# Megvii-CSG/MegReader

Measured on AMD Instinct MI355X. Metric: training images/sec, CRNN-CTC 32x128 crops, batch 256 per GPU, higher is better.
Workload: dtype bf16; 1 GPU; CRNN + 1D-CTC training step (BASELINE.json configs[1]): 32x128 crops, T=33, C=38, Adam; global_batch=256, per_gpu_batch=256, parallelism=dp1, launch=hipGraph replay

## Files before the change

include/megreader_hip.h:

```cpp
#ifndef MEGREADER_HIP_H
#define MEGREADER_HIP_H

#include <hip/hip_runtime_api.h>

#ifdef __cplusplus
extern "C" {
#endif

#define MR_ABI_VERSION 3
#define MR_DTYPE_F32 0
#define MR_DTYPE_BF16 1

const char* mr_last_error(void);
int mr_abi_version(void);
int mr_phase_timer(int on);
int mr_phase_read(int id, double* total_ms, double* total_work);
int mr_init(void);

typedef struct mr_tuning {
  int nt_variant;
  int nt_deep;
  int nt_big;
  int nt_p8;
  int nt_force_bm;
// ... 48 lines not shown
                int NA, int NB, int row_perm_h, float* colsum, float* colsum2, hipStream_t stream);

int mr_tn_defer(int on);
int mr_tn_pending(void);
int mr_tn_discard(void);
int mr_tn_flush(hipStream_t stream);
int mr_tn_flush_beside(hipStream_t stream);

int mr_conv2d_fwd(int dtype, const void* x, const void* w_krsc, const float* bias, void* y, int relu, int Nimg,
                  int H, int W, int Cin, int ldx, int Cout, int ldy, int R, int S, int sh, int sw, int ph, int pw,
                  int dh, int dw, int Ho, int Wo, hipStream_t stream);
int mr_conv2d_fwd_pool_ok(int dtype, int Nimg, int H, int W, int Cin, int ldx, int Cout, int R, int S, int sh, int sw, int ph, int pw,
                          int dh, int dw, int Ho, int Wo, int pkh, int pkw, int psh, int psw, int pph, int ppw);
int mr_conv2d_fwd_pool(int dtype, const void* x, const void* w_krsc, const float* bias, void* y_pool, unsigned char* idx, int relu,
                       int Nimg, int H, int W, int Cin, int ldx, int Cout, int R, int S, int sh, int sw, int ph, int pw, int dh,
                       int dw, int Ho, int Wo, int pkh, int pkw, int psh, int psw, int pph, int ppw, int PHo, int PWo,
                       hipStream_t stream);
int mr_conv2d_fwd_stats(int dtype, const void* x, const void* w_krsc, const float* bias, void* y, double* bn_sums, int Nimg,
                        int H, int W, int Cin, int ldx, int Cout, int R, int S, int sh, int sw, int ph, int pw, int dh,
                        int dw, int Ho, int Wo, hipStream_t stream);
int mr_conv2d_dgrad(int dtype, const void* dy, const void* w_crsk, void* dx, int Nimg, int H, int W, int Cin,
                    int lddx, int Cout, int lddy, int R, int S, int sh, int sw, int ph, int pw, int dh, int dw,
                    int Ho, int Wo, hipStream_t stream);
int mr_conv2d_dgrad_add(int dtype, const void* dy, const void* w_crsk, void* dx, const void* addend, int Nimg, int H, int W,
                        int Cin, int lddx, int Cout, int lddy, int R, int S, int sh, int sw, int ph, int pw, int dh, int dw,
                        int Ho, int Wo, hipStream_t stream);
int mr_conv2d_dgrad_bnb(int dtype, const void* dy, const void* w_crsk, void* dx, const void* addend, const void* bn_x,
                        const void* bn_y, const float* bn_mean, const float* bn_rstd, double* bn_sums, int* produced,
                        int Nimg, int H, int W, int Cin, int lddx, int Cout, int lddy, int R, int S, int sh, int sw, int ph,
                        int pw, int dh, int dw, int Ho, int Wo, hipStream_t stream);
int mr_conv2d_wgrad(int dtype, const void* dy, const void* x, float* dw_krsc, float* dbias, int Nimg, int H, int W,
                    int Cin, int ldx, int Cout, int lddy, int R, int S, int sh, int sw, int ph, int pw, int dh,
                    int dw, int Ho, int Wo, hipStream_t stream);
int mr_conv2d_wgrad_tab(int dtype, const void* dy, const void* x, float* dw_krsc, float* dbias, int N, int H, int W,
                        int Cin, int ldx, int Cout, int lddy, int R, int S, int sh, int sw, int ph, int pw, int dh,
                        int dw, int Ho, int Wo, void* rowtab, int build, hipStream_t stream);

long long mr_db_loss_ws_bytes(void);
int mr_db_head_tail_fwd(int dtype, const void* xb, const void* xt, float* binary, float* thresh, float* tbinary, long long n,
                        float k, hipStream_t stream);
int mr_db_head_tail_bwd(int dtype, const float* binary, const float* thresh, const float* tbinary, const float* gb,
                        const float* gt, const float* gtb, void* dxb, void* dxt, long long n, float k, hipStream_t stream);
int mr_db_loss_fwd(const float* binary, const float* thresh, const float* tbinary, const float* gt, const float* mask,
                   const float* tmap, const float* tmask, float* negloss, void* ws, float* out, int N, long long HW,
                   float negative_ratio, float eps, float l1_scale, float bce_scale, hipStream_t stream);
int mr_db_loss_bwd(const float* binary, const float* thresh, const float* tbinary, const float* gt, const float* mask,
// ... 380 lines not shown
```

megreader_amd/backbones/crnn.py:

```python
import torch.nn as nn

from ..nn import Conv2d, BatchNorm2d, MaxPool2d, FusedReLU
from ..nn import functional as F


class _Stem(nn.Sequential):

    def forward(self, input):
        conv, pool = self[0][0], self[1]
        if F.stem_eligible(input, conv.weight, conv.stride, conv.padding, conv.dilation, _pair(pool.kernel_size),
                           _pair(pool.stride), _pair(pool.padding)):
            return F.stem_conv_relu_pool(input, conv.weight, conv.bias)
        return super().forward(input)


class _ConvReluPool(nn.Sequential):

    def forward(self, input):
        conv, pool = self[0][0], self[1]
        if F.conv_relu_pool_eligible(input, conv.weight, conv.stride, conv.padding, conv.dilation, _pair(pool.kernel_size),
                                     _pair(pool.stride), _pair(pool.padding)):
            return F.conv_relu_pool(input, conv.weight, conv.bias, conv.padding, _pair(pool.kernel_size), _pair(pool.stride),
                                    _pair(pool.padding))
        return super().forward(input)
# ... 5 lines not shown

class CRNN(nn.Module):

    def __init__(self, imgH, nc, nclass, nh):
        super(CRNN, self).__init__()
        assert imgH % 16 == 0, 'imgH has to be a multiple of 16'

        self.kernels = [3, 3, 3, 3, 3, 3, 2]
        self.paddings = [1, 1, 1, 1, 1, 1, 0]
        self.strides = [1, 1, 1, 1, 1, 1, 1]
        self.channels = [64, 128, 256, 256, 512, 512, 512, nc]

        conv0 = _Stem(self._make_layer(0, pooled=True), MaxPool2d((2, 2), relu_input=True))
        conv1 = _ConvReluPool(self._make_layer(1, pooled=True), MaxPool2d((2, 2), relu_input=True))
        conv2 = self._make_layer(2, True)
        conv3 = _ConvReluPool(self._make_layer(3, pooled=True), MaxPool2d((2, 2), (2, 1), (0, 1), relu_input=True))
        conv4 = self._make_layer(4, True)
        conv5 = _ConvReluPool(self._make_layer(5, pooled=True), MaxPool2d((2, 2), (2, 1), (0, 1), relu_input=True))
        conv6 = self._make_layer(6, True)

        self.cnn = nn.Sequential(conv0, conv1, conv2, conv3, conv4, conv5, conv6)
        conv3[0][0].sole_consumer_of_bn = True
        conv5[0][0].sole_consumer_of_bn = True

    def _make_layer(self, i, batch_normalization=False, pooled=False):
        in_channel = self.channels[i - 1]
        out_channel = self.channels[i]
        layer = list()
        layer.append(Conv2d(in_channel, out_channel, self.kernels[i], self.strides[i], self.paddings[i],
                            fuse_relu=not batch_normalization,
                            relu_grad_downstream=pooled and not batch_normalization))
        if batch_normalization:
            layer.append(BatchNorm2d(out_channel))
        else:
            layer.append(FusedReLU())
        return nn.Sequential(*layer)

    def forward(self, input):
        return self.cnn(input)


def crnn_backbone(imgH=32, nc=3, nclass=37, nh=256):
    return CRNN(imgH, nc, nclass, nh)
```

megreader_amd/csrc/gemm_conv.hip:

```cpp
#include "igemm_core.h"
#include "igemm_p8.h"
#include "tn_taps.h"
#include "nt32.h"
#include "device.h"
#include "../../include/megreader_hip.h"

#include <algorithm>
#include <mutex>
#include <vector>

namespace mr {

static bool aligned16(const void* p) { return (((uintptr_t)p) & 15) == 0; }

#define g_nt_variant MR_TUNE(nt_variant)
#define g_nt_deep MR_TUNE(nt_deep)

struct BnbRequest { const void* x; const void* y; const float* mean; const float* rstd; };
struct NtEpilogue {
  const float* bias = nullptr;
  int relu = 0;
  const void* addend = nullptr;
  double* stats = nullptr;
  BnbRequest bnb = {nullptr, nullptr, nullptr, nullptr};
// ... 560 lines not shown
  }
  const TileChoice tw = nt_tile(M, N);
  if (tw.bm == 128 && tw.bn == 128 && (MR_TUNE(nt_wide8) & 1) && N % 128 == 0) {
    const int t = fit(128);
    if (t == 128) { *tile_rows = t; return 8; }
  }
  return 0;
}

template <int WM, int WN, int TM, int TN>
static int launch_nt_pool(const NtArgs& a, const ConvGeom& g, const EpiPool<bf16_t>& epi, hipStream_t stream) {
  constexpr int BM = WM * TM * 16, BN = WN * TN * 16;
  constexpr size_t lds_stage = 2 * (size_t)(BM + BN) * 128, lds_tile = (size_t)BM * BN * 2;
  constexpr size_t lds = lds_stage > lds_tile ? lds_stage : lds_tile;
  auto kern = igemm_nt_big_kernel<bf16_t, WM, WN, TM, TN, 2, EpiPool<bf16_t>>;
  if (const int rc = ensure_dynamic_lds(kern, lds)) return rc;
  const int tiles_m = cdiv(a.M, a.tile_rows), tiles_n = cdiv(a.N, BN);
  const int grid = cdiv(tiles_m, 8) * 8 * tiles_n;
  hipLaunchKernelGGL(kern, dim3(grid), dim3(64 * WM * WN), lds, stream, a, g, epi);
  MR_CHECK_LAUNCH();
  return MR_OK;
}


extern "C" {

int mr_init(void) {
  const int rc = tuning_from_env();
  if (rc != MR_OK) return rc;
  if (!zero_page()) { set_error("mr_init: zero page allocation failed"); return MR_ERR_LAUNCH; }
  return MR_OK;
}

#ifdef MR_ABLATION
int mr_set_tn_abl(int mask) {
  const int old = g_tn_abl;
  g_tn_abl = mask;
  return old;
}
int mr_set_tn_taps_abl(int mask) { return taps_set_abl(mask); }
#endif

int mr_set_tn_taps_workspace(void* ws, long long bytes) {
  MR_CHECK_ARG((ws == nullptr) == (bytes == 0) && bytes >= 0 && (((uintptr_t)ws) & 15) == 0,
               "mr_set_tn_taps_workspace: bad workspace");
  taps_set_workspace(ws, bytes);
// ... 184 lines not shown
                        hipStream_t stream) {
  MR_CHECK_ARG(dtype == MR_F32 || dtype == MR_BF16, "mr_conv2d_dgrad: bad dtype %d", dtype);
  const int vec = dtype == MR_F32 ? 4 : 8;
  MR_CHECK_ARG(Cout % vec == 0 && lddy % vec == 0, "mr_conv2d_dgrad: Cout/lddy must be multiples of %d", vec);
  MR_CHECK_ARG(aligned16(dy) && aligned16(w_crsk), "mr_conv2d_dgrad: dy and w must be 16-byte aligned");
  NtArgs a;
  a.A = dy; a.B = w_crsk; a.M = Nimg * H * W; a.N = Cin; a.K = R * S * Cout; a.lda = 0; a.ldb = R * S * Cout; a.zero = nullptr;
  ConvGeom g;
  fill_geom(g, 2, Ho, Wo, Cout, lddy, H, W, R, S, sh, sw, ph, pw, dh, dw);
  if (R * S <= 32 && sh == 1 && sw == 1) {
    if (dtype == MR_F32) return dispatch_nt_store<float, 2>(a, g, dx, lddx, o, stream);
    return dispatch_nt_store<bf16_t, 2>(a, g, dx, lddx, o, stream);
  }
  if (dtype == MR_F32) return dispatch_nt_store<float, 1>(a, g, dx, lddx, o, stream);
  return dispatch_nt_store<bf16_t, 1>(a, g, dx, lddx, o, stream);
}
int mr_conv2d_dgrad(int dtype, const void* dy, const void* w_crsk, void* dx, int Nimg, int H, int W, int Cin,
                    int lddx, int Cout, int lddy, int R, int S, int sh, int sw, int ph, int pw, int dh, int dw,
                    int Ho, int Wo, hipStream_t stream) {
  NtEpilogue o;
  return conv2d_dgrad(dtype, dy, w_crsk, dx, o, Nimg, H, W, Cin, lddx, Cout, lddy, R, S, sh, sw, ph, pw, dh, dw, Ho, Wo, stream);
}

int mr_conv2d_dgrad_add(int dtype, const void* dy, const void* w_crsk, void* dx, const void* addend, int Nimg, int H, int W,
                        int Cin, int lddx, int Cout, int lddy, int R, int S, int sh, int sw, int ph, int pw, int dh, int dw,
                        int Ho, int Wo, hipStream_t stream) {
  NtEpilogue o;
  o.addend = addend;
  return conv2d_dgrad(dtype, dy, w_crsk, dx, o, Nimg, H, W, Cin, lddx, Cout, lddy, R, S, sh, sw, ph, pw, dh, dw, Ho, Wo, stream);
}

int mr_conv2d_dgrad_bnb(int dtype, const void* dy, const void* w_crsk, void* dx, const void* addend, const void* bn_x,
                        const void* bn_y, const float* bn_mean, const float* bn_rstd, double* bn_sums, int* produced,
                        int Nimg, int H, int W, int Cin, int lddx, int Cout, int lddy, int R, int S, int sh, int sw, int ph,
                        int pw, int dh, int dw, int Ho, int Wo, hipStream_t stream) {
  MR_CHECK_ARG(bn_x && bn_mean && bn_rstd && bn_sums && produced, "mr_conv2d_dgrad_bnb: null BatchNorm operand");
  MR_CHECK_ARG(lddx == Cin, "mr_conv2d_dgrad_bnb: dx must be dense (lddx == Cin), like the BatchNorm's tensors");
  MR_CHECK_ARG(aligned16(bn_x) && (bn_y == nullptr || aligned16(bn_y)), "mr_conv2d_dgrad_bnb: bn_x / bn_y must be 16-byte aligned");
  NtEpilogue o;
  o.addend = addend;
  o.stats = bn_sums;
  o.bnb = BnbRequest{bn_x, bn_y, bn_mean, bn_rstd};
  const int rc = conv2d_dgrad(dtype, dy, w_crsk, dx, o, Nimg, H, W, Cin, lddx, Cout, lddy, R, S, sh, sw, ph, pw, dh, dw, Ho, Wo,
                              stream);
  *produced = o.stats_missed ? 0 : 1;
  return rc;
// ... 57 lines not shown
```

megreader_amd/csrc/igemm_core.h:

```cpp
#pragma once
#include "common.h"
#include <type_traits>

namespace mr {

struct ConvGeom {
  int Hg, Wg, Cg, ldg;
  int Hm, Wm;
  int R, S, sh, sw, ph, pw, dh, dw;
  int mode;
};

__device__ __forceinline__ bool conv_src(const ConvGeom& g, int hm, int wm, int r, int s, int& hi, int& wi) {
  if (g.mode == 1) {
    hi = hm * g.sh - g.ph + r * g.dh;
    wi = wm * g.sw - g.pw + s * g.dw;
  } else {
    int hn = hm + g.ph - r * g.dh;
    int wn = wm + g.pw - s * g.dw;
    if (hn < 0 || wn < 0) return false;
    if (g.sh == 1 && g.sw == 1) {
      hi = hn;
      wi = wn;
    } else {
// ... 18 lines not shown
#pragma unroll
    for (int j = 0; j < 4; ++j) acc = __builtin_amdgcn_mfma_f32_16x16x4f32(a[j], b[j], acc, 0, 0, 0);
  }
};

struct NtArgs {
  const void* A;
  const void* B;
  int M, N, K;
  long long lda;
  int ldb;
  const void* zero;
  int m_begin = 0;
  int ksplit = 1;
  void* ws = nullptr;
  int tile_rows = 0;
};
constexpr int NT_SPLIT_TICKETS = 4096;

__device__ __forceinline__ uint4 ldg16(const void* p) { return *(const uint4*)p; }

template <typename Epi> struct EpiHasStats { static constexpr bool value = false; };
template <typename Epi> struct EpiIsPool { static constexpr bool value = false; };
__device__ __forceinline__ float row16_sum(float v) {
#define MR_ROW_ROR(V, N) __builtin_bit_cast(float, __builtin_amdgcn_update_dpp(0, __builtin_bit_cast(int, V), 0x120 + (N), 0xf, 0xf, false))
  v += MR_ROW_ROR(v, 8);
  v += MR_ROW_ROR(v, 4);
  v += MR_ROW_ROR(v, 2);
  v += MR_ROW_ROR(v, 1);
#undef MR_ROW_ROR
  return v;
}
template <typename T, int CNT> struct EpiColStats {
  float s[4 * CNT], q[4 * CNT];
  __device__ __forceinline__ void init() {
#pragma unroll
    for (int e = 0; e < 4 * CNT; ++e) s[e] = q[e] = 0.f;
  }
  template <typename Epi> __device__ __forceinline__ void add(const Epi& epi, int m, int n, const f32x4* v) {
    if (m >= epi.M) return;
    if constexpr (Epi::kBnb) {
      const long long row = (long long)m * epi.ldc + n;
#pragma unroll
      for (int i = 0; i < CNT; ++i)
#pragma unroll
        for (int j = 0; j < 4; ++j) {
// ... 1192 lines not shown
                  }
                  first = false;
                }
            }
          T o[8];
#pragma unroll
          for (int e = 0; e < 8; ++e) o[e] = from_f32<T>(best[e]);
          const long long q = (((long long)nimg * epi.PHo + h / kh) * epi.PWo + pwi) * epi.ldc + n0 + c * 8;
          *(uint4*)(epi.C + q) = *(const uint4*)o;
          *(uint2*)(epi.idx + q) = *(const uint2*)bi;
        }
        pwi += PSTEP;
        while (pwi >= epi.PWo) {
          pwi -= epi.PWo;
          ++pr;
          h += kh;
          if (h >= epi.Ho) { h -= epi.Ho; ++nimg; }
        }
      }
    };
    if (epi.kh == 2 && epi.kw == 2) pool_one(std::integral_constant<int, 2>{}, std::integral_constant<int, 2>{});
    else pool_one(std::integral_constant<int, 0>{}, std::integral_constant<int, 0>{});
    return;
  } else {
    constexpr bool FLAGSHIP = (WM == 2 && WN == 4 && TM == 8 && TN == 4) || (WM == 1 && WN == 8 && TM == 17 && TN == 2);
    constexpr int EPI_PATHS = FLAGSHIP ? NT_EPI_STORE : (TN == 2 && !(WM == 4 && TM == 3)) ? (NT_EPI_PLAIN | NT_EPI_ADD) : 0;
    if constexpr (EPI_PATHS != 0) {
      if (nt_epilogue_interior<T, TM, TN, EPI_PATHS>(epi, m0 + wm_ * WTM, n0 + wn_ * WTN, l15, lg,
                                                      [&](int i, int j) -> f32x4 { return acc[i][j]; }))
        return;
    }
  EpiColStats<T, TN> cst;
  bool with_stats = false;
  if constexpr (EpiHasStats<Epi>::value) with_stats = epi.stats != nullptr;
  if (with_stats) cst.init();
#pragma unroll
  for (int j = 0; j < TM; ++j) {
    f32x4 run[TN];
#pragma unroll
    for (int i = 0; i < TN; ++i) run[i] = acc[i][j];
    if constexpr (EpiHasStats<Epi>::value)
      if (with_stats) cst.add(epi, m0 + wm_ * WTM + j * 16 + l15, n0 + wn_ * WTN + lg * (4 * TN), run);
    epi.template store_run<TN>(m0 + wm_ * WTM + j * 16 + l15, n0 + wn_ * WTN + lg * (4 * TN), run);
  }
  if constexpr (EpiHasStats<Epi>::value)
    if (with_stats) cst.flush(epi, n0 + wn_ * WTN + lg * (4 * TN), l15);
  }
}

template <typename T> struct EpiPool {
  T* C;
  unsigned char* idx;
  long long ldc;
  const float* bias;
  int relu;
  int M, N;
  int Nimg, Ho, Wo, kh, kw, sw, pw, PHo, PWo;
};
template <typename T> struct EpiIsPool<EpiPool<T>> { static constexpr bool value = true; };

template <typename T> struct EpiStore {
  T* C;
  long long ldc;
  const float* bias;
  int relu;
  int M, N;
  int vec_ok;
  double* stats = nullptr;
  int stats_ncopy = 1;
  const T* addend = nullptr;
  static constexpr bool kBnb = false;
  __device__ __forceinline__ void operator()(int m, int n, f32x4 v) const {
    if (m >= M || n >= N) return;
    if (bias) {
#pragma unroll
      for (int j = 0; j < 4; ++j)
        if (n + j < N) v[j] += bias[n + j];
    }
    if (addend) {
      const T* a = addend + (long long)m * ldc + n;
#pragma unroll
      for (int j = 0; j < 4; ++j)
// ... 932 lines not shown
```

megreader_amd/nn/functional.py:

```python
import ctypes
import os

import torch
from torch.autograd import Function

from .. import get_compute_dtype
from . import prep
from .._lib import call, dtype_code, load, ptr, require_cuda, vec_of

_ESIZE = {torch.float32: 4, torch.bfloat16: 2}


def _ceil_to(x, m):
    return (x + m - 1) // m * m


def grad_sink(param, physical_shape=None):
    sink = getattr(param, "_mr_grad_sink", None)
    if sink is None or sink.dtype != torch.float32 or not sink.is_cuda:
        return None
    if param.grad is None or param.grad.data_ptr() != sink.data_ptr():
        return None
    if physical_shape == "strided":
        return sink
# ... 264 lines not shown
    K, C, R, S = weight.shape
    dev = weight.device

    def build(old):
        if old is None:
            alloc = torch.zeros if Kp != K else torch.empty
            w_krsc = alloc((Kp, R, S, Cp), dtype=dtype, device=dev)
            w_crsk = alloc((C, R, S, Kp), dtype=dtype, device=dev) if need_dx else None
            bias_p = torch.zeros((Kp,), dtype=torch.float32, device=dev) if (bias is not None and Kp != K) else None
        else:
            w_krsc, w_crsk, bias_p = old
        jobs = [prep.conv_job(ptr(weight), weight.stride(), ptr(w_krsc), ptr(w_crsk), K, C, R, S, Cp, Kp)]
        if bias_p is not None:
            jobs.append(prep.bias_job(ptr(bias), 0, ptr(bias_p), K, 0))
        return (w_krsc, w_crsk, bias_p), jobs

    w_krsc, w_crsk, bias_p = prep.prepared((weight, bias), ("conv", Cp, Kp, bool(need_dx)), build, dtype)
    return w_krsc, w_crsk, (bias_p if bias_p is not None else bias)


class Conv2dFn(Function):
    @staticmethod
    def forward(ctx, x, weight, bias, stride, padding, dilation, relu, relu_grad_downstream=False, bn_sums=None,
                fork=False, bnb_link=None):
        require_cuda(x, weight, bias)
        ctx.bnb_link = bnb_link
        dtype = get_compute_dtype()
        dt = dtype_code(dtype)
        v = vec_of(dtype)
        xi = to_internal(x, dtype)
        N, H, W, Cp = xi.shape
        K, C, R, S = weight.shape
        if C > Cp or weight.dtype != torch.float32:
            raise RuntimeError("conv weight %s does not match input channels %d" % (tuple(weight.shape), Cp))
        Kp = _ceil_to(K, v)
        sh, sw = stride
        ph, pw = padding
        dh, dw = dilation
        Ho, Wo = _conv_out(H, R, sh, ph, dh), _conv_out(W, S, sw, pw, dw)
        need_dx = ctx.needs_input_grad[0]
        if need_dx and Cp != C:
            raise RuntimeError("input gradient requested for a channel-padded convolution input")
        w_krsc, w_crsk, bias_k = _conv_operands(weight, bias, dtype, Cp, Kp, need_dx)
        y = torch.empty((N, Ho, Wo, Kp), dtype=dtype, device=x.device)
        if bn_sums is not None and not relu and Kp == K:
            call("mr_conv2d_fwd_stats", dt, ptr(xi), ptr(w_krsc), ptr(bias_k), ptr(y), ptr(bn_sums), N, H, W, Cp, Cp, Kp,
                 R, S, sh, sw, ph, pw, dh, dw, Ho, Wo)
        else:
            call("mr_conv2d_fwd", dt, ptr(xi), ptr(w_krsc), ptr(bias_k), ptr(y), int(relu), N, H, W, Cp, Cp, Kp, Kp, R,
# ... 27 lines not shown
            call("mr_relu_bwd", dt, ptr(g), ptr(y), ptr(gm), g.numel())
            g = gm
        dx = dwt = db = None
        if ctx.needs_input_grad[0]:
            dxi = torch.empty((N, H, W, C), dtype=dtype, device=g.device)
            ga = None
            if g_fork is not None:
                ga = _grad_internal(g_fork, dtype)
                if tuple(ga.shape) != (N, H, W, C) or not ga.is_contiguous():
                    ga = ga.contiguous()
            link = ctx.bnb_link
            fused_bnb = False
            if link is not None and link.xi is not None and link.dtype == dtype and tuple(link.xi.shape) == (N, H, W, C) and \
                    BNB_EPILOGUE:
                sums = ZeroArena.take(g.device, load().mr_bn_scratch_doubles(C))
                if sums is not None:
                    produced = ctypes.c_int(0)
                    call("mr_conv2d_dgrad_bnb", dt, ptr(g), ptr(w_crsk), ptr(dxi), ptr(ga), ptr(link.xi), ptr(link.y),
                         ptr(link.mean), ptr(link.rstd), ptr(sums), ctypes.byref(produced), N, H, W, C, C, Kp, Kp, R, S, sh,
                         sw, ph, pw, dh, dw, Ho, Wo)
                    fused_bnb = True
                    if produced.value:
                        link.sums, link.grad_ptr = sums, dxi.data_ptr()
            if fused_bnb:
                pass
            elif ga is not None:
                call("mr_conv2d_dgrad_add", dt, ptr(g), ptr(w_crsk), ptr(dxi), ptr(ga), N, H, W, C, C, Kp, Kp, R, S, sh, sw,
                     ph, pw, dh, dw, Ho, Wo)
            elif POINTWISE_STRIDED_DGRAD and R == 1 and S == 1 and (sh > 1 or sw > 1) and ph == 0 and pw == 0:
                dxs = torch.empty((N, Ho, Wo, C), dtype=dtype, device=g.device)
                call("mr_conv2d_dgrad", dt, ptr(g), ptr(w_crsk), ptr(dxs), N, Ho, Wo, C, C, Kp, Kp, 1, 1, 1, 1, 0, 0, 1, 1, Ho,
                     Wo)
                call("mr_scatter_strided", dt, ptr(dxs), ptr(dxi), N, H, W, C, sh, sw, Ho, Wo)
            else:
                call("mr_conv2d_dgrad", dt, ptr(g), ptr(w_crsk), ptr(dxi), N, H, W, C, C, Kp, Kp, R, S, sh, sw, ph, pw,
                     dh, dw, Ho, Wo)
            dx = dxi.permute(0, 3, 1, 2)
        elif g_fork is not None:
            raise RuntimeError("conv2d_fork: the forked input received a gradient but the convolution input needs none")
        weight_p, bias_p = ctx.params
        want_db = ctx.has_bias and ctx.needs_input_grad[2]
        w_sink = grad_sink(weight_p, (K, R, S, C)) if (ctx.needs_input_grad[1] and Cp == C) else None
        b_sink = grad_sink(bias_p, (K,)) if want_db else None
        Kw = K if (w_sink is not None or b_sink is not None) else Kp
        if want_db:
            db = b_sink if b_sink is not None else torch.zeros((Kp,), dtype=torch.float32, device=g.device)
        if ctx.needs_input_grad[1]:
            gw = w_sink if w_sink is not None else torch.zeros((Kp, R, S, Cp), dtype=torch.float32, device=g.device)
            tab, build = (None, 0)
            if dtype == torch.bfloat16 and R * S <= 32:
                tab, build = _wgrad_rowtab(g.device, (N, H, W, Cp, R, S, sh, sw, ph, pw, dh, dw, Ho, Wo), Kw % 8 == 0)
            def wgrad_launch():
                call("mr_conv2d_wgrad_tab", dt, ptr(g), ptr(xi), ptr(gw), ptr(db) if want_db else 0, N, H, W, Cp, Cp, Kw,
                     Kp, R, S, sh, sw, ph, pw, dh, dw, Ho, Wo, ptr(tab), build)
            if _wgrad(wgrad_launch, w_sink is not None and (not want_db or b_sink is not None), (g, xi, tab),
                      [weight_p] + ([bias_p] if want_db else [])):
                return dx, None, None, None, None, None, None, None, None, None, None
            if w_sink is not None:
                dwt = None
                notify_grad_ready(weight_p)
            else:
                if Cp != C or Kp != K:
                    gw = gw[:K, :, :, :C]
                dwt = gw.permute(0, 3, 1, 2)
        elif want_db:
            call("mr_colsum", dt, ptr(g), ptr(db), N * Ho * Wo, Kw, Kp, 0)
        if want_db:
            if b_sink is not None:
                db = None
                notify_grad_ready(bias_p)
            elif Kp != K:
                db = db[:K]
        return dx, dwt, db, None, None, None, None, None, None, None, None


POINTWISE_STRIDED_DGRAD = os.environ.get("MEGREADER_POINTWISE_STRIDED_DGRAD", "1") != "0"

BNB_EPILOGUE = os.environ.get("MEGREADER_BNB_EPILOGUE", "0") == "1"


_DIST_GUARD = {"done": False}


def _no_resident_grids_beside_collectives():
    if _DIST_GUARD["done"]:
        return
    import torch.distributed as dist
    if dist.is_available() and dist.is_initialized():
        from ..runtime import no_resident_grid_kernels_beside_collectives
        no_resident_grid_kernels_beside_collectives(dist.get_world_size())
        _DIST_GUARD["done"] = True


class BnBwdLink(object):
    __slots__ = ("xi", "y", "mean", "rstd", "dtype", "sums", "grad_ptr")

    def __init__(self):
        self.xi = self.y = self.mean = self.rstd = self.dtype = self.sums = self.grad_ptr = None


class BnStatsHandoff(object):
    __slots__ = ("sums", "data_ptr", "dtype", "P", "C")

    def __init__(self, sums, data_ptr, dtype, P, C):
        self.sums, self.data_ptr, self.dtype, self.P, self.C = sums, data_ptr, dtype, P, C


def conv2d(x, weight, bias=None, stride=(1, 1), padding=(0, 0), dilation=(1, 1), relu=False,
           relu_grad_downstream=False, bn_stats=False, fork=False, sole_consumer_of_bn=False):
    sums = None
    if bn_stats and not relu and x.is_cuda:
        K = weight.shape[0]
        if K % vec_of(get_compute_dtype()) == 0:
            sums = ZeroArena.take(x.device, load().mr_bn_scratch_doubles(K))
    want_fork = bool(fork)
    fork = want_fork and x.requires_grad and torch.is_grad_enabled()
    link = getattr(x, "_mr_bnb_link", None) if (sole_consumer_of_bn and x.requires_grad and torch.is_grad_enabled()) else None
    y = Conv2dFn.apply(x, weight, bias, tuple(stride), tuple(padding), tuple(dilation), bool(relu),
                       bool(relu_grad_downstream), sums, fork, link)
    x_fork = x
    if fork:
        y, x_fork = y
    if sums is not None:
        y._mr_bn_sums = BnStatsHandoff(sums, y.data_ptr(), get_compute_dtype(), y.shape[0] * y.shape[2] * y.shape[3],
                                       y.shape[1])
    return (y, x_fork) if want_fork else y


class BatchNormFn(Function):
    @staticmethod
    def forward(ctx, x, gamma, beta, running_mean, running_var, training, momentum, eps, relu, residual,
                num_batches_tracked=None, pre=None, link=None):
        require_cuda(x, gamma, beta)
        dtype = get_compute_dtype()
        dt = dtype_code(dtype)
        xi = to_internal(x, dtype)
        N, H, W, C = xi.shape
        if C != gamma.numel():
            raise RuntimeError("BatchNorm2d: channel mismatch (%d vs %d)" % (C, gamma.numel()))
        P = N * H * W
        ri = to_internal(residual, dtype) if residual is not None else None
        y = torch.empty_like(xi)
# ... 218 lines not shown
        if want_db:
            db = b_sink if b_sink is not None else torch.zeros((64,), dtype=torch.float32, device=g.device)
        if dw is not None or db is not None:
            ws = torch.empty((load().mr_stem_bwd_workspace(C),), dtype=torch.float32, device=g.device)
            sk, sc, sr, ss = dw.stride() if dw is not None else (0, 0, 0, 0)
            call("mr_stem_bwd", dtype_code(dtype), ptr(g), ptr(code), ptr(x), ptr(ws), ptr(dw), sk, sc, sr, ss, ptr(db),
                 N, C, H, W)
        if w_sink is not None:
            notify_grad_ready(weight_p)
            dw = None
        if b_sink is not None:
            notify_grad_ready(bias_p)
            db = None
        return None, dw, db


def stem_conv_relu_pool(x, weight, bias):
    return StemConvReluPoolFn.apply(x, weight, bias)


class ConvReluPoolFn(Function):

    @staticmethod
    def forward(ctx, x, weight, bias, padding, pool_kernel, pool_stride, pool_padding):
        require_cuda(x, weight, bias)
        dtype = get_compute_dtype()
        dt = dtype_code(dtype)
        xi = to_internal(x, dtype)
        N, H, W, Cp = xi.shape
        K, C, R, S = weight.shape
        ph, pw = padding
        Ho, Wo = _conv_out(H, R, 1, ph, 1), _conv_out(W, S, 1, pw, 1)
        kh, kw = pool_kernel
        psh, psw = pool_stride
        pph, ppw = pool_padding
        PHo, PWo = (Ho + 2 * pph - kh) // psh + 1, (Wo + 2 * ppw - kw) // psw + 1
        need_dx = ctx.needs_input_grad[0]
        w_krsc, w_crsk, bias_k = _conv_operands(weight, bias, dtype, Cp, K, need_dx)
        y = torch.empty((N, PHo, PWo, K), dtype=dtype, device=x.device)
        idx = torch.empty((N, PHo, PWo, K), dtype=torch.uint8, device=x.device)
        call("mr_conv2d_fwd_pool", dt, ptr(xi), ptr(w_krsc), ptr(bias_k), ptr(y), ptr(idx), 1, N, H, W, Cp, Cp, K, R, S, 1, 1, ph, pw,
             1, 1, Ho, Wo, kh, kw, psh, psw, pph, ppw, PHo, PWo)
        ctx.save_for_backward(xi, w_crsk, idx, y)
        ctx.params = (weight, bias)
        ctx.geom = (N, H, W, Cp, C, K, K, R, S, 1, 1, ph, pw, 1, 1, Ho, Wo)
        ctx.pool = (kh, kw, psh, psw, pph, ppw, PHo, PWo)
        ctx.has_bias = bias is not None
        ctx.dtype = dtype
        return y.permute(0, 3, 1, 2)

    @staticmethod
    def backward(ctx, gy):
        xi, w_crsk, idx, y = ctx.saved_tensors
        N, H, W, Cp, C, K, Kp, R, S, sh, sw, ph, pw, dh, dw, Ho, Wo = ctx.geom
        kh, kw, psh, psw, pph, ppw, PHo, PWo = ctx.pool
        dtype = ctx.dtype
        g = _grad_internal(gy, dtype)
        dz = torch.empty((N, Ho, Wo, K), dtype=dtype, device=g.device)
        call("mr_maxpool_bwd", dtype_code(dtype), ptr(g), ptr(idx), ptr(y), ptr(dz), N, Ho, Wo, K, kh, kw, psh, psw, pph, ppw,
             PHo, PWo)

        class _ConvCtx(object):
            pass
        c = _ConvCtx()
        c.saved_tensors = (xi, w_crsk, None)
        c.geom, c.dtype, c.params, c.has_bias = ctx.geom, dtype, ctx.params, ctx.has_bias
        c.relu, c.bnb_link = False, None
        c.needs_input_grad = (ctx.needs_input_grad[0], ctx.needs_input_grad[1], ctx.needs_input_grad[2]) + (False,) * 8
        grads = Conv2dFn.backward(c, dz.permute(0, 3, 1, 2))
        return grads[0], grads[1], grads[2], None, None, None, None


def conv_relu_pool_eligible(x, weight, stride, padding, dilation, pool_kernel, pool_stride, pool_padding):
    if not x.is_cuda or get_compute_dtype() != torch.bfloat16 or tuple(stride) != (1, 1) or tuple(dilation) != (1, 1):
        return False
    if os.environ.get("MEGREADER_CONV_POOL", "1") == "0":
        return False
    N, C, H, W = x.shape
    K, Cw, R, S = weight.shape
    if C != Cw or C % 8 != 0 or K % 8 != 0:
        return False
    ph, pw = padding
    Ho, Wo = _conv_out(H, R, 1, ph, 1), _conv_out(W, S, 1, pw, 1)
    return bool(load().mr_conv2d_fwd_pool_ok(dtype_code(torch.bfloat16), N, H, W, C, C, K, R, S, 1, 1, ph, pw, 1, 1, Ho, Wo,
                                             pool_kernel[0], pool_kernel[1], pool_stride[0], pool_stride[1],
                                             pool_padding[0], pool_padding[1]))


def conv_relu_pool(x, weight, bias, padding, pool_kernel, pool_stride, pool_padding):
    return ConvReluPoolFn.apply(x, weight, bias, tuple(padding), tuple(pool_kernel), tuple(pool_stride), tuple(pool_padding))


class MaxPoolFn(Function):
    @staticmethod
    def forward(ctx, x, kernel, stride, padding, relu_input=False):
        require_cuda(x)
        dtype = get_compute_dtype()
        dt = dtype_code(dtype)
        xi = to_internal(x, dtype)
        N, H, W, C = xi.shape
        kh, kw = kernel
        sh, sw = stride
        ph, pw = padding
        Ho, Wo = (H + 2 * ph - kh) // sh + 1, (W + 2 * pw - kw) // sw + 1
        y = torch.empty((N, Ho, Wo, C), dtype=dtype, device=x.device)
        idx = torch.empty((N, Ho, Wo, C), dtype=torch.uint8, device=x.device)
        call("mr_maxpool_fwd", dt, ptr(xi), ptr(y), ptr(idx), N, H, W, C, kh, kw, sh, sw, ph, pw, Ho, Wo)
        ctx.save_for_backward(idx, y if relu_input else None)
        ctx.geom = (N, H, W, C, kh, kw, sh, sw, ph, pw, Ho, Wo)
        ctx.dtype = dtype
        return y.permute(0, 3, 1, 2)

    @staticmethod
    def backward(ctx, gy):
        idx, relu_y = ctx.saved_tensors
        N, H, W, C, kh, kw, sh, sw, ph, pw, Ho, Wo = ctx.geom
        dtype = ctx.dtype
        g = _grad_internal(gy, dtype)
        dx = torch.empty((N, H, W, C), dtype=dtype, device=g.device)
        call("mr_maxpool_bwd", dtype_code(dtype), ptr(g), ptr(idx), ptr(relu_y), ptr(dx), N, H, W, C, kh, kw, sh, sw,
             ph, pw, Ho, Wo)
        return dx.permute(0, 3, 1, 2), None, None, None, None


def max_pool2d(x, kernel, stride=None, padding=(0, 0), relu_input=False):
    stride = kernel if stride is None else stride
    return MaxPoolFn.apply(x, tuple(kernel), tuple(stride), tuple(padding), bool(relu_input))


class MapToSequenceFn(Function):
    @staticmethod
    def forward(ctx, x):
        require_cuda(x)
        dtype = get_compute_dtype()
        xi = to_internal(x, dtype)
        N, H, W, C = xi.shape
        if H != 1:
            raise AssertionError("the height of conv must be 1")
        out = torch.empty((W, N, C), dtype=dtype, device=x.device)
        call("mr_permute_021", dtype_code(dtype), ptr(xi), ptr(out), N, W, C)
        ctx.shape = (N, W, C)
        ctx.dtype = dtype
        return out

    @staticmethod
    def backward(ctx, g):
        N, W, C = ctx.shape
        dtype = ctx.dtype
        if g.dtype != dtype or not g.is_contiguous():
            g = g.to(dtype).contiguous()
# ... 814 lines not shown
```

megreader_amd/nn/modules.py:

```python
import math

import torch
import torch.nn as nn

from . import functional as F


BN_EPILOGUE = __import__("os").environ.get("MEGREADER_BN_EPILOGUE", "1") != "0"


FORK_RESIDUAL = __import__("os").environ.get("MEGREADER_FORK_RESIDUAL", "1") != "0"


def _pair(v):
    return tuple(v) if isinstance(v, (tuple, list)) else (v, v)


class Conv2d(nn.Conv2d):

    def __init__(self, *args, fuse_relu=False, relu_grad_downstream=False, **kwargs):
        super().__init__(*args, **kwargs)
        if self.groups != 1 or self.padding_mode != "zeros" or isinstance(self.padding, str):
            raise NotImplementedError("megreader_amd.nn.Conv2d supports groups=1 and explicit zero padding only")
        self.fuse_relu = fuse_relu
        self.relu_grad_downstream = relu_grad_downstream and fuse_relu
        self.weight.data = self.weight.data.contiguous(memory_format=torch.channels_last)

    feeds_batch_norm = False
    sole_consumer_of_bn = False
    sole_consumer_when_forked = False

    def forward(self, x):
        y = F.conv2d(x, self.weight, self.bias, self.stride, self.padding, self.dilation, self.fuse_relu,
                     self.relu_grad_downstream, bn_stats=self.feeds_batch_norm and self.training and BN_EPILOGUE,
                     sole_consumer_of_bn=self.sole_consumer_of_bn)
        y._mr_producer = self
        return y

    def forward_fork(self, x):
        if not FORK_RESIDUAL:
            y = F.conv2d(x, self.weight, self.bias, self.stride, self.padding, self.dilation, self.fuse_relu,
                         self.relu_grad_downstream, bn_stats=self.feeds_batch_norm and self.training and BN_EPILOGUE)
            y._mr_producer = self
            return y, x
        y, xr = F.conv2d(x, self.weight, self.bias, self.stride, self.padding, self.dilation, self.fuse_relu,
                         self.relu_grad_downstream, bn_stats=self.feeds_batch_norm and self.training and BN_EPILOGUE,
                         fork=True, sole_consumer_of_bn=self.sole_consumer_when_forked)
        y._mr_producer = self
        return y, xr


class FusedReLU(nn.Module):

    def forward(self, x):
        return x


class BatchNorm2d(nn.BatchNorm2d):
# ... 80 lines not shown
```

Measured before the change: 109,800 images/s.

## Fuse maxpool backward scatter into the following conv's dgrad epilogue

Result: no change. 110,600 images/s (median of 6 runs) (+0.6%).

```diff
diff --git a/include/megreader_hip.h b/include/megreader_hip.h
--- a/include/megreader_hip.h
+++ b/include/megreader_hip.h
@@ -94,6 +94,14 @@
 int mr_conv2d_dgrad(int dtype, const void* dy, const void* w_crsk, void* dx, int Nimg, int H, int W, int Cin,
                     int lddx, int Cout, int lddy, int R, int S, int sh, int sw, int ph, int pw, int dh, int dw,
                     int Ho, int Wo, hipStream_t stream);
+int mr_set_dgrad_unpool(int on);
+int mr_conv2d_dgrad_unpool_ok(int dtype, int Nimg, int H, int W, int Cin, int lddx, int Cout, int lddy, int R, int S, int sh, int sw,
+                              int ph, int pw, int dh, int dw, int Ho, int Wo, int pkh, int pkw, int psh, int psw, int pph, int ppw,
+                              int H_full, int W_full);
+int mr_conv2d_dgrad_unpool(int dtype, const void* dy, const void* w_crsk, void* dx_full, const unsigned char* idx, const void* relu_y,
+                           int Nimg, int H, int W, int Cin, int lddx, int Cout, int lddy, int R, int S, int sh, int sw, int ph, int pw,
+                           int dh, int dw, int Ho, int Wo, int pkh, int pkw, int psh, int psw, int pph, int ppw, int H_full, int W_full,
+                           hipStream_t stream);
 int mr_conv2d_dgrad_add(int dtype, const void* dy, const void* w_crsk, void* dx, const void* addend, int Nimg, int H, int W,
                         int Cin, int lddx, int Cout, int lddy, int R, int S, int sh, int sw, int ph, int pw, int dh, int dw,
                         int Ho, int Wo, hipStream_t stream);
diff --git a/megreader_amd/backbones/crnn.py b/megreader_amd/backbones/crnn.py
--- a/megreader_amd/backbones/crnn.py
+++ b/megreader_amd/backbones/crnn.py
@@ -51,6 +51,9 @@
         self.cnn = nn.Sequential(conv0, conv1, conv2, conv3, conv4, conv5, conv6)
         conv3[0][0].sole_consumer_of_bn = True
         conv5[0][0].sole_consumer_of_bn = True
+        conv2[0].sole_consumer_of_pool = True
+        conv4[0].sole_consumer_of_pool = True
+        conv6[0].sole_consumer_of_pool = True
 
     def _make_layer(self, i, batch_normalization=False, pooled=False):
         in_channel = self.channels[i - 1]
diff --git a/megreader_amd/csrc/gemm_conv.hip b/megreader_amd/csrc/gemm_conv.hip
--- a/megreader_amd/csrc/gemm_conv.hip
+++ b/megreader_amd/csrc/gemm_conv.hip
@@ -606,6 +606,46 @@
   return MR_OK;
 }
 
+static int g_dgrad_unpool = 1;
+
+static int dgrad_unpool_plan(int M, int N, int K, int Cg, int PWo, int* tile_rows) {
+  if (!__atomic_load_n(&g_dgrad_unpool, __ATOMIC_RELAXED) || g_nt_variant != 2 || forced_tile().bm || (Cg % 64) != 0 ||
+      MR_TUNE(nt_m32) >= 2 || N % 8 != 0 || PWo <= 0 || M % PWo != 0)
+    return 0;
+  int tile = 0;
+  if (g_big_mode == 7 || g_big_mode == 8) tile = g_big_mode;
+  else if (g_big_mode != 0 || nt_big_choice(M, N, K) != 0 || nt_head_rows(M, N, K) > 0) return 0;
+  else if (nt_use_288x128(M, N, K)) tile = 7;
+  else {
+    const TileChoice tw = nt_tile(M, N);
+    if (!((MR_TUNE(nt_wide8) & 1) && tw.bm == 128 && tw.bn == 128)) return 0;
+    tile = 8;
+  }
+  const int bm = tile == 7 ? 288 : 128;
+  const int t = (bm / PWo) * PWo;
+  if (t <= 0) return 0;
+  const long long slots = (long long)num_cus() * (tile == 7 ? 1 : 2);
+  const long long tiles_n = cdiv(N, 128);
+  const long long plain = cdiv(M, bm) * tiles_n, fused = cdiv(M, t) * tiles_n;
+  if ((fused + slots - 1) / slots > (plain + slots - 1) / slots) return 0;
+  *tile_rows = t;
+  return tile;
+}
+
+template <int WM, int WN, int TM, int TN>
+static int launch_nt_unpool(const NtArgs& a, const ConvGeom& g, const EpiUnpool<bf16_t>& epi, hipStream_t stream) {
+  constexpr int BM = WM * TM * 16, BN = WN * TN * 16;
+  constexpr size_t lds_stage = 2 * (size_t)(BM + BN) * 128, lds_tile = (size_t)BM * BN * 3;
+  constexpr size_t lds = lds_stage > lds_tile ? lds_stage : lds_tile;
+  auto kern = igemm_nt_big_kernel<bf16_t, WM, WN, TM, TN, 2, EpiUnpool<bf16_t>>;
+  if (const int rc = ensure_dynamic_lds(kern, lds)) return rc;
+  const int tiles_m = cdiv(a.M, a.tile_rows), tiles_n = cdiv(a.N, BN);
+  const int grid = cdiv(tiles_m, 8) * 8 * tiles_n;
+  hipLaunchKernelGGL(kern, dim3(grid), dim3(64 * WM * WN), lds, stream, a, g, epi);
+  MR_CHECK_LAUNCH();
+  return MR_OK;
+}
+
 
 extern "C" {
 
@@ -836,6 +876,56 @@
   return conv2d_dgrad(dtype, dy, w_crsk, dx, o, Nimg, H, W, Cin, lddx, Cout, lddy, R, S, sh, sw, ph, pw, dh, dw, Ho, Wo, stream);
 }
 
+int mr_set_dgrad_unpool(int on) { return __atomic_exchange_n(&g_dgrad_unpool, on ? 1 : 0, __ATOMIC_RELAXED); }
+
+static int dgrad_unpool_geom(int dtype, int Nimg, int H, int W, int Cin, int lddx, int Cout, int lddy, int R, int S, int sh, int sw,
+                             int ph, int pw, int dh, int dw, int Ho, int Wo, int pkh, int pkw, int psh, int psw, int pph, int ppw,
+                             int H_full, int W_full, NtArgs& a, ConvGeom& g) {
+  (void)ph; (void)pw; (void)dh; (void)dw;
+  if (dtype != MR_BF16 || Nimg <= 0 || H <= 0 || W <= 0 || R * S > 32 || sh != 1 || sw != 1 || Cin % 8 != 0 || lddx != Cin ||
+      Cout % 8 != 0 || lddy % 8 != 0)
+    return 0;
+  if (pkh < 1 || pkw < 1 || psw < 1 || pkh != psh || pph != 0 || ppw < 0 || H_full != pkh * H || pkw > 2 * psw || pkh * pkw > 255 ||
+      W_full < 1 || W_full + 2 * ppw < pkw || W != (W_full + 2 * ppw - pkw) / psw + 1)
+    return 0;
+  const long long full_bytes = (long long)Nimg * H_full * W_full * Cin * 2, pooled_bytes = (long long)Nimg * H * W * Cin * 2;
+  if (full_bytes >= (1ll << 31) || pooled_bytes >= (1ll << 31)) return 0;
+  a.M = Nimg * H * W; a.N = Cin; a.K = R * S * Cout; a.lda = 0; a.ldb = R * S * Cout; a.zero = nullptr;
+  fill_geom(g, 2, Ho, Wo, Cout, lddy, H, W, R, S, sh, sw, ph, pw, dh, dw);
+  if (!nt_fits_buffer<bf16_t>(a, g, 2)) return 0;
+  return dgrad_unpool_plan(a.M, a.N, a.K, Cout, W, &a.tile_rows);
+}
+
+int mr_conv2d_dgrad_unpool_ok(int dtype, int Nimg, int H, int W, int Cin, int lddx, int Cout, int lddy, int R, int S, int sh, int sw,
+                              int ph, int pw, int dh, int dw, int Ho, int Wo, int pkh, int pkw, int psh, int psw, int pph, int ppw,
+                              int H_full, int W_full) {
+  NtArgs a;
+  ConvGeom g;
+  return dgrad_unpool_geom(dtype, Nimg, H, W, Cin, lddx, Cout, lddy, R, S, sh, sw, ph, pw, dh, dw, Ho, Wo, pkh, pkw, psh, psw, pph, ppw,
+                           H_full, W_full, a, g) ? 1 : 0;
+}
+
+int mr_conv2d_dgrad_unpool(int dtype, const void* dy, const void* w_crsk, void* dx_full, const unsigned char* idx, const void* relu_y,
+                           int Nimg, int H, int W, int Cin, int lddx, int Cout, int lddy, int R, int S, int sh, int sw, int ph, int pw,
+                           int dh, int dw, int Ho, int Wo, int pkh, int pkw, int psh, int psw, int pph, int ppw, int H_full, int W_full,
+                           hipStream_t stream) {
+  NtArgs a;
+  ConvGeom g;
+  const int plan = dgrad_unpool_geom(dtype, Nimg, H, W, Cin, lddx, Cout, lddy, R, S, sh, sw, ph, pw, dh, dw, Ho, Wo, pkh, pkw, psh, psw,
+                                     pph, ppw, H_full, W_full, a, g);
+  MR_CHECK_ARG(plan != 0, "mr_conv2d_dgrad_unpool: geometry not served (ask mr_conv2d_dgrad_unpool_ok)");
+  MR_CHECK_ARG(dy && w_crsk && dx_full && idx, "mr_conv2d_dgrad_unpool: null operand");
+  MR_CHECK_ARG(aligned16(dy) && aligned16(w_crsk) && aligned16(dx_full) && aligned16(relu_y) && ((uintptr_t)idx & 7) == 0,
+               "mr_conv2d_dgrad_unpool: alignment");
+  a.A = dy; a.B = w_crsk; a.zero = zero_page();
+  if (!a.zero) { set_error("zero page allocation failed"); return MR_ERR_LAUNCH; }
+  EpiUnpool<bf16_t> epi;
+  epi.C = (bf16_t*)dx_full; epi.idx = idx; epi.relu_y = (const bf16_t*)relu_y; epi.ldc = Cin; epi.M = a.M; epi.N = Cin;
+  epi.PWo = W; epi.Wf = W_full; epi.kh = pkh; epi.kw = pkw; epi.sw = psw; epi.pw = ppw;
+  if (plan == 7) return launch_nt_unpool<2, 4, 9, 2>(a, g, epi, stream);
+  return launch_nt_unpool<2, 4, 4, 2>(a, g, epi, stream);
+}
+
 int mr_conv2d_dgrad_add(int dtype, const void* dy, const void* w_crsk, void* dx, const void* addend, int Nimg, int H, int W,
                         int Cin, int lddx, int Cout, int lddy, int R, int S, int sh, int sw, int ph, int pw, int dh, int dw,
                         int Ho, int Wo, hipStream_t stream) {
diff --git a/megreader_amd/csrc/igemm_core.h b/megreader_amd/csrc/igemm_core.h
--- a/megreader_amd/csrc/igemm_core.h
+++ b/megreader_amd/csrc/igemm_core.h
@@ -64,6 +64,7 @@
 
 template <typename Epi> struct EpiHasStats { static constexpr bool value = false; };
 template <typename Epi> struct EpiIsPool { static constexpr bool value = false; };
+template <typename Epi> struct EpiIsUnpool { static constexpr bool value = false; };
 __device__ __forceinline__ float row16_sum(float v) {
 #define MR_ROW_ROR(V, N) __builtin_bit_cast(float, __builtin_amdgcn_update_dpp(0, __builtin_bit_cast(int, V), 0x120 + (N), 0xf, 0xf, false))
   v += MR_ROW_ROR(v, 8);
@@ -1302,6 +1303,123 @@
     if (epi.kh == 2 && epi.kw == 2) pool_one(std::integral_constant<int, 2>{}, std::integral_constant<int, 2>{});
     else pool_one(std::integral_constant<int, 0>{}, std::integral_constant<int, 0>{});
     return;
+  } else if constexpr (EpiIsUnpool<Epi>::value) {
+    static_assert(sizeof(T) == 2, "unpool epilogue: bf16 only");
+    constexpr int CH = BN / 8;
+    static_assert((CH & (CH - 1)) == 0 && (4 * TN) % 8 == 0, "unpool epilogue: tile width / lane run in whole 16-byte chunks");
+    __syncthreads();
+    uint2* scode = (uint2*)(smem + BM * CH);
+    {
+      constexpr int NQ = TM * (TN / 2);
+      const bool with_mask = epi.relu_y != nullptr;
+      uint2 cd[NQ];
+      uint4 yv[NQ];
+#pragma unroll
+      for (int j = 0; j < TM; ++j) {
+        const int r = wm_ * WTM + j * 16 + l15;
+#pragma unroll
+        for (int q = 0; q < TN / 2; ++q) {
+          const int cc = (wn_ * WTN + lg * (4 * TN)) / 8 + q;
+          const bool ok = r < trows && m0 + r < epi.M && n0 + cc * 8 < epi.N;
+          const long long go = (long long)(m0 + r) * epi.ldc + n0 + cc * 8;
+          cd[j * (TN / 2) + q] = ok ? *(const uint2*)(epi.idx + go) : make_uint2(~0u, ~0u);
+          yv[j * (TN / 2) + q] = (ok && with_mask) ? *(const uint4*)(epi.relu_y + go) : make_uint4(0, 0, 0, 0);
+        }
+      }
+#pragma unroll
+      for (int j = 0; j < TM; ++j) {
+        const int r = wm_ * WTM + j * 16 + l15;
+#pragma unroll
+        for (int q = 0; q < TN / 2; ++q) {
+          T o[8];
+#pragma unroll
+          for (int e = 0; e < 8; ++e) o[e] = from_f32<T>(acc[2 * q + e / 4][j][e % 4]);
+          uint2 cv = cd[j * (TN / 2) + q];
+          if (with_mask) {
+            const T* py = (const T*)&yv[j * (TN / 2) + q];
+            unsigned char* pc = (unsigned char*)&cv;
+#pragma unroll
+            for (int e = 0; e < 8; ++e)
+              if (!(to_f32(py[e]) > 0.f)) pc[e] = 255;
+          }
+          const int cc = (wn_ * WTN + lg * (4 * TN)) / 8 + q;
+          smem[r * CH + (cc ^ (r & (CH - 1)))] = *(const uint4*)o;
+          scode[r * CH + (cc ^ (r & (CH - 1)))] = cv;
+        }
+      }
+    }
+    __syncthreads();
+    int prows = trows / epi.PWo;
+    if ((epi.M - m0) / epi.PWo < prows) prows = (epi.M - m0) / epi.PWo;
+    const int prow0 = m0 / epi.PWo;
+    constexpr int PSTEP = 64 * NW / CH;
+    const int c = tid % CH;
+    int pr = (tid / CH) / epi.Wf, w = (tid / CH) - pr * epi.Wf;
+    if (n0 + c * 8 >= epi.N) return;
+    const long long ch0 = n0 + c * 8;
+    auto unpool = [&](auto fast_tag) {
+      constexpr bool FAST = decltype(fast_tag)::value;
+      for (; pr < prows;) {
+        if constexpr (FAST) {
+          const int sshift = epi.sw - 1;
+          float a0[8], a1[8];
+#pragma unroll
+          for (int e = 0; e < 8; ++e) a0[e] = a1[e] = 0.f;
+#pragma unroll
+          for (int jx = 0; jx < 2; ++jx) {
+            const int wn = w + epi.pw - jx;
+            const int wo = wn >> sshift;
+            if (wn < 0 || (wo << sshift) != wn || wo >= epi.PWo) continue;
+            const int r = pr * epi.PWo + wo;
+            const uint4 gv = smem[r * CH + (c ^ (r & (CH - 1)))];
+            const T* pg = (const T*)&gv;
+            const uint2 cv = scode[r * CH + (c ^ (r & (CH - 1)))];
+            const unsigned char* code = (const unsigned char*)&cv;
+#pragma unroll
+            for (int e = 0; e < 8; ++e) {
+              if (code[e] == jx) a0[e] += to_f32(pg[e]);
+              if (code[e] == 2 + jx) a1[e] += to_f32(pg[e]);
+            }
+          }
+          T o0[8], o1[8];
+#pragma unroll
+          for (int e = 0; e < 8; ++e) { o0[e] = from_f32<T>(a0[e]); o1[e] = from_f32<T>(a1[e]); }
+          const long long d = ((long long)(prow0 + pr) * 2 * epi.Wf + w) * epi.ldc + ch0;
+          *(uint4*)(epi.C + d) = *(const uint4*)o0;
+          *(uint4*)(epi.C + d + (long long)epi.Wf * epi.ldc) = *(const uint4*)o1;
+        } else {
+          for (int i = 0; i < epi.kh; ++i) {
+            float a0[8];
+#pragma unroll
+            for (int e = 0; e < 8; ++e) a0[e] = 0.f;
+            for (int jx = 0; jx < epi.kw; ++jx) {
+              const int wn = w + epi.pw - jx;
+              if (wn < 0) continue;
+              const int wo = wn / epi.sw;
+              if (wo * epi.sw != wn || wo >= epi.PWo) continue;
+              const int r = pr * epi.PWo + wo;
+              const uint4 gv = smem[r * CH + (c ^ (r & (CH - 1)))];
+              const T* pg = (const T*)&gv;
+              const uint2 cv = scode[r * CH + (c ^ (r & (CH - 1)))];
+              const unsigned char* code = (const unsigned char*)&cv;
+              const int want = i * epi.kw + jx;
+#pragma unroll
+              for (int e = 0; e < 8; ++e)
+                if (code[e] == want) a0[e] += to_f32(pg[e]);
+            }
+            T o0[8];
+#pragma unroll
+            for (int e = 0; e < 8; ++e) o0[e] = from_f32<T>(a0[e]);
+            *(uint4*)(epi.C + (((long long)(prow0 + pr) * epi.kh + i) * epi.Wf + w) * epi.ldc + ch0) = *(const uint4*)o0;
+          }
+        }
+        w += PSTEP;
+        while (w >= epi.Wf) { w -= epi.Wf; ++pr; }
+      }
+    };
+    if (epi.kh == 2 && epi.kw == 2 && (epi.sw == 1 || epi.sw == 2)) unpool(std::true_type{});
+    else unpool(std::false_type{});
+    return;
   } else {
     constexpr bool FLAGSHIP = (WM == 2 && WN == 4 && TM == 8 && TN == 4) || (WM == 1 && WN == 8 && TM == 17 && TN == 2);
     constexpr int EPI_PATHS = FLAGSHIP ? NT_EPI_STORE : (TN == 2 && !(WM == 4 && TM == 3)) ? (NT_EPI_PLAIN | NT_EPI_ADD) : 0;
@@ -1338,6 +1456,16 @@
   int Nimg, Ho, Wo, kh, kw, sw, pw, PHo, PWo;
 };
 template <typename T> struct EpiIsPool<EpiPool<T>> { static constexpr bool value = true; };
+
+template <typename T> struct EpiUnpool {
+  T* C;
+  const unsigned char* idx;
+  const T* relu_y;
+  long long ldc;
+  int M, N;
+  int PWo, Wf, kh, kw, sw, pw;
+};
+template <typename T> struct EpiIsUnpool<EpiUnpool<T>> { static constexpr bool value = true; };
 
 template <typename T> struct EpiStore {
   T* C;
diff --git a/megreader_amd/nn/functional.py b/megreader_amd/nn/functional.py
--- a/megreader_amd/nn/functional.py
+++ b/megreader_amd/nn/functional.py
@@ -310,9 +310,11 @@
 class Conv2dFn(Function):
     @staticmethod
     def forward(ctx, x, weight, bias, stride, padding, dilation, relu, relu_grad_downstream=False, bn_sums=None,
-                fork=False, bnb_link=None):
+                fork=False, bnb_link=None, unpool_link=None):
         require_cuda(x, weight, bias)
         ctx.bnb_link = bnb_link
+        ctx.unpool_link = unpool_link
+        ctx.unpool_x = x if unpool_link is not None else None
         dtype = get_compute_dtype()
         dt = dtype_code(dtype)
         v = vec_of(dtype)
@@ -386,8 +388,18 @@
                     fused_bnb = True
                     if produced.value:
                         link.sums, link.grad_ptr = sums, dxi.data_ptr()
+            ul = getattr(ctx, "unpool_link", None)
             if fused_bnb:
                 pass
+            elif ul is not None and ga is None and _dgrad_unpool_ok(ul, ctx.unpool_x, dtype, ctx.geom):
+                kh, kw, psh, psw, pph, ppw = ul.pool
+                Hf, Wf = ul.full_hw
+                dz = torch.empty((N, Hf, Wf, C), dtype=dtype, device=g.device)
+                call("mr_conv2d_dgrad_unpool", dt, ptr(g), ptr(w_crsk), ptr(dz), ptr(ul.idx), ptr(ul.relu_y), N, H, W, C, C, Kp,
+                     Kp, R, S, sh, sw, ph, pw, dh, dw, Ho, Wo, kh, kw, psh, psw, pph, ppw, Hf, Wf)
+                if UNPOOL_POISON_PLACEHOLDER:
+                    dxi.fill_(float("nan"))
+                ul.dx_full, ul.grad_ptr = dz, dxi.data_ptr()
             elif ga is not None:
                 call("mr_conv2d_dgrad_add", dt, ptr(g), ptr(w_crsk), ptr(dxi), ptr(ga), N, H, W, C, C, Kp, Kp, R, S, sh, sw,
                      ph, pw, dh, dw, Ho, Wo)
@@ -419,7 +431,7 @@
                      Kp, R, S, sh, sw, ph, pw, dh, dw, Ho, Wo, ptr(tab), build)
             if _wgrad(wgrad_launch, w_sink is not None and (not want_db or b_sink is not None), (g, xi, tab),
                       [weight_p] + ([bias_p] if want_db else [])):
-                return dx, None, None, None, None, None, None, None, None, None, None
+                return dx, None, None, None, None, None, None, None, None, None, None, None
             if w_sink is not None:
                 dwt = None
                 notify_grad_ready(weight_p)
@@ -435,7 +447,7 @@
                 notify_grad_ready(bias_p)
             elif Kp != K:
                 db = db[:K]
-        return dx, dwt, db, None, None, None, None, None, None, None, None
+        return dx, dwt, db, None, None, None, None, None, None, None, None, None
 
 
 POINTWISE_STRIDED_DGRAD = os.environ.get("MEGREADER_POINTWISE_STRIDED_DGRAD", "1") != "0"
@@ -470,8 +482,38 @@
         self.sums, self.data_ptr, self.dtype, self.P, self.C = sums, data_ptr, dtype, P, C
 
 
+class UnpoolLink(object):
+    __slots__ = ("idx", "relu_y", "pool", "full_hw", "dtype", "dx_full", "grad_ptr")
+
+    def __init__(self):
+        self.idx = self.relu_y = self.pool = self.full_hw = self.dtype = self.dx_full = self.grad_ptr = None
+
+    def fill(self, idx, relu_y, pool, full_hw, dtype):
+        self.idx, self.relu_y, self.pool, self.full_hw, self.dtype = idx, relu_y, tuple(pool), tuple(full_hw), dtype
+
+    def take(self, gy):
+        dz = self.dx_full if (self.dx_full is not None and self.grad_ptr == gy.data_ptr()) else None
+        self.idx = self.relu_y = self.dx_full = self.grad_ptr = None
+        return dz
+
+
+UNPOOL_POISON_PLACEHOLDER = False
+
+
+def _dgrad_unpool_ok(link, x, dtype, geom):
+    N, H, W, Cp, C, K, Kp, R, S, sh, sw, ph, pw, dh, dw, Ho, Wo = geom
+    if link.idx is None or dtype != torch.bfloat16 or link.dtype != dtype or Cp != C or tuple(link.idx.shape) != (N, H, W, C):
+        return False
+    if x is None or x.retains_grad or getattr(x, "_backward_hooks", None):
+        return False
+    kh, kw, psh, psw, pph, ppw = link.pool
+    Hf, Wf = link.full_hw
+    return bool(load().mr_conv2d_dgrad_unpool_ok(dtype_code(dtype), N, H, W, C, C, Kp, Kp, R, S, sh, sw, ph, pw, dh, dw, Ho, Wo,
+                                                 kh, kw, psh, psw, pph, ppw, Hf, Wf))
+
+
 def conv2d(x, weight, bias=None, stride=(1, 1), padding=(0, 0), dilation=(1, 1), relu=False,
-           relu_grad_downstream=False, bn_stats=False, fork=False, sole_consumer_of_bn=False):
+           relu_grad_downstream=False, bn_stats=False, fork=False, sole_consumer_of_bn=False, sole_consumer_of_pool=False):
     sums = None
     if bn_stats and not relu and x.is_cuda:
         K = weight.shape[0]
@@ -480,8 +522,10 @@
     want_fork = bool(fork)
     fork = want_fork and x.requires_grad and torch.is_grad_enabled()
     link = getattr(x, "_mr_bnb_link", None) if (sole_consumer_of_bn and x.requires_grad and torch.is_grad_enabled()) else None
+    ulink = getattr(x, "_mr_unpool_link", None) if (sole_consumer_of_pool and not fork and x.requires_grad and
+                                                     torch.is_grad_enabled()) else None
     y = Conv2dFn.apply(x, weight, bias, tuple(stride), tuple(padding), tuple(dilation), bool(relu),
-                       bool(relu_grad_downstream), sums, fork, link)
+                       bool(relu_grad_downstream), sums, fork, link, ulink)
     x_fork = x
     if fork:
         y, x_fork = y
@@ -746,7 +790,7 @@
 class ConvReluPoolFn(Function):
 
     @staticmethod
-    def forward(ctx, x, weight, bias, padding, pool_kernel, pool_stride, pool_padding):
+    def forward(ctx, x, weight, bias, padding, pool_kernel, pool_stride, pool_padding, unpool_link=None):
         require_cuda(x, weight, bias)
         dtype = get_compute_dtype()
         dt = dtype_code(dtype)
@@ -769,6 +813,9 @@
         ctx.params = (weight, bias)
         ctx.geom = (N, H, W, Cp, C, K, K, R, S, 1, 1, ph, pw, 1, 1, Ho, Wo)
         ctx.pool = (kh, kw, psh, psw, pph, ppw, PHo, PWo)
+        ctx.unpool_link = unpool_link
+        if unpool_link is not None:
+            unpool_link.fill(idx, y, (kh, kw, psh, psw, pph, ppw), (Ho, Wo), dtype)
         ctx.has_bias = bias is not None
         ctx.dtype = dtype
         return y.permute(0, 3, 1, 2)
@@ -779,20 +826,22 @@
         N, H, W, Cp, C, K, Kp, R, S, sh, sw, ph, pw, dh, dw, Ho, Wo = ctx.geom
         kh, kw, psh, psw, pph, ppw, PHo, PWo = ctx.pool
         dtype = ctx.dtype
-        g = _grad_internal(gy, dtype)
-        dz = torch.empty((N, Ho, Wo, K), dtype=dtype, device=g.device)
-        call("mr_maxpool_bwd", dtype_code(dtype), ptr(g), ptr(idx), ptr(y), ptr(dz), N, Ho, Wo, K, kh, kw, psh, psw, pph, ppw,
-             PHo, PWo)
+        dz = ctx.unpool_link.take(gy) if ctx.unpool_link is not None else None
+        if dz is None:
+            g = _grad_internal(gy, dtype)
+            dz = torch.empty((N, Ho, Wo, K), dtype=dtype, device=g.device)
+            call("mr_maxpool_bwd", dtype_code(dtype), ptr(g), ptr(idx), ptr(y), ptr(dz), N, Ho, Wo, K, kh, kw, psh, psw, pph, ppw,
+                 PHo, PWo)
 
         class _ConvCtx(object):
             pass
         c = _ConvCtx()
         c.saved_tensors = (xi, w_crsk, None)
         c.geom, c.dtype, c.params, c.has_bias = ctx.geom, dtype, ctx.params, ctx.has_bias
-        c.relu, c.bnb_link = False, None
+        c.relu, c.bnb_link, c.unpool_link, c.unpool_x = False, None, None, None
         c.needs_input_grad = (ctx.needs_input_grad[0], ctx.needs_input_grad[1], ctx.needs_input_grad[2]) + (False,) * 8
         grads = Conv2dFn.backward(c, dz.permute(0, 3, 1, 2))
-        return grads[0], grads[1], grads[2], None, None, None, None
+        return grads[0], grads[1], grads[2], None, None, None, None, None
 
 
 def conv_relu_pool_eligible(x, weight, stride, padding, dilation, pool_kernel, pool_stride, pool_padding):
@@ -811,13 +860,21 @@
                                              pool_padding[0], pool_padding[1]))
 
 
+def _new_unpool_link(*needs_grad):
+    return UnpoolLink() if (torch.is_grad_enabled() and any(t is not None and t.requires_grad for t in needs_grad)) else None
+
+
 def conv_relu_pool(x, weight, bias, padding, pool_kernel, pool_stride, pool_padding):
-    return ConvReluPoolFn.apply(x, weight, bias, tuple(padding), tuple(pool_kernel), tuple(pool_stride), tuple(pool_padding))
+    link = _new_unpool_link(x, weight, bias)
+    out = ConvReluPoolFn.apply(x, weight, bias, tuple(padding), tuple(pool_kernel), tuple(pool_stride), tuple(pool_padding), link)
+    if link is not None and link.idx is not None:
+        out._mr_unpool_link = link
+    return out
 
 
 class MaxPoolFn(Function):
     @staticmethod
-    def forward(ctx, x, kernel, stride, padding, relu_input=False):
+    def forward(ctx, x, kernel, stride, padding, relu_input=False, unpool_link=None):
         require_cuda(x)
         dtype = get_compute_dtype()
         dt = dtype_code(dtype)
@@ -833,6 +890,9 @@
         ctx.save_for_backward(idx, y if relu_input else None)
         ctx.geom = (N, H, W, C, kh, kw, sh, sw, ph, pw, Ho, Wo)
         ctx.dtype = dtype
+        ctx.unpool_link = unpool_link
+        if unpool_link is not None:
+            unpool_link.fill(idx, y if relu_input else None, (kh, kw, sh, sw, ph, pw), (H, W), dtype)
         return y.permute(0, 3, 1, 2)
 
     @staticmethod
@@ -840,16 +900,22 @@
         idx, relu_y = ctx.saved_tensors
         N, H, W, C, kh, kw, sh, sw, ph, pw, Ho, Wo = ctx.geom
         dtype = ctx.dtype
-        g = _grad_internal(gy, dtype)
-        dx = torch.empty((N, H, W, C), dtype=dtype, device=g.device)
-        call("mr_maxpool_bwd", dtype_code(dtype), ptr(g), ptr(idx), ptr(relu_y), ptr(dx), N, H, W, C, kh, kw, sh, sw,
-             ph, pw, Ho, Wo)
-        return dx.permute(0, 3, 1, 2), None, None, None, None
+        dx = ctx.unpool_link.take(gy) if ctx.unpool_link is not None else None
+        if dx is None:
+            g = _grad_internal(gy, dtype)
+            dx = torch.empty((N, H, W, C), dtype=dtype, device=g.device)
+            call("mr_maxpool_bwd", dtype_code(dtype), ptr(g), ptr(idx), ptr(relu_y), ptr(dx), N, H, W, C, kh, kw, sh, sw,
+                 ph, pw, Ho, Wo)
+        return dx.permute(0, 3, 1, 2), None, None, None, None, None
 
 
 def max_pool2d(x, kernel, stride=None, padding=(0, 0), relu_input=False):
     stride = kernel if stride is None else stride
-    return MaxPoolFn.apply(x, tuple(kernel), tuple(stride), tuple(padding), bool(relu_input))
+    link = _new_unpool_link(x) if relu_input else None
+    out = MaxPoolFn.apply(x, tuple(kernel), tuple(stride), tuple(padding), bool(relu_input), link)
+    if link is not None and link.idx is not None:
+        out._mr_unpool_link = link
+    return out
 
 
 class MapToSequenceFn(Function):
diff --git a/megreader_amd/nn/modules.py b/megreader_amd/nn/modules.py
--- a/megreader_amd/nn/modules.py
+++ b/megreader_amd/nn/modules.py
@@ -28,12 +28,13 @@
 
     feeds_batch_norm = False
     sole_consumer_of_bn = False
+    sole_consumer_of_pool = False
     sole_consumer_when_forked = False
 
     def forward(self, x):
         y = F.conv2d(x, self.weight, self.bias, self.stride, self.padding, self.dilation, self.fuse_relu,
                      self.relu_grad_downstream, bn_stats=self.feeds_batch_norm and self.training and BN_EPILOGUE,
-                     sole_consumer_of_bn=self.sole_consumer_of_bn)
+                     sole_consumer_of_bn=self.sole_consumer_of_bn, sole_consumer_of_pool=self.sole_consumer_of_pool)
         y._mr_producer = self
         return y
 
```
